# NeSC-IV/sage-icp

Hardware: AMD Instinct MI355X
Metric: ICP frames/sec (120k-pt scan vs 1M-pt map) (higher is better)
Workload: dtype f64

## Files before the change

### sage-icp_amd/csrc/capi_run.hip

```cpp
#include "capi_internal.h"

namespace sageicp_impl {

Rccl g_rccl;
static std::mutex g_rccl_mu;


int load_rccl() {
    std::lock_guard<std::mutex> lk(g_rccl_mu);
    if (g_rccl.h) return SAGEICP_OK;
    const char *names[] = {"librccl.so.1", "librccl.so", "/opt/rocm/lib/librccl.so.1"};
    void *h = nullptr;
    for (const char *n : names) {
        h = dlopen(n, RTLD_NOW | RTLD_NOLOAD | RTLD_GLOBAL);
        if (h) break;
    }
    for (int i = 0; i < 3 && !h; ++i) h = dlopen(names[i], RTLD_NOW | RTLD_GLOBAL);
    if (!h) return fail(SAGEICP_ERR_RCCL, std::string("cannot load librccl: ") + dlerror());
    g_rccl.GetUniqueId = reinterpret_cast<decltype(g_rccl.GetUniqueId)>(dlsym(h, "ncclGetUniqueId"));
    g_rccl.CommInitRank = reinterpret_cast<decltype(g_rccl.CommInitRank)>(dlsym(h, "ncclCommInitRank"));
    g_rccl.CommDestroy = reinterpret_cast<decltype(g_rccl.CommDestroy)>(dlsym(h, "ncclCommDestroy"));
    g_rccl.AllReduce = reinterpret_cast<decltype(g_rccl.AllReduce)>(dlsym(h, "ncclAllReduce"));
    g_rccl.GetErrorString = reinterpret_cast<decltype(g_rccl.GetErrorString)>(dlsym(h, "ncclGetErrorString"));
    g_rccl.CommCount = reinterpret_cast<decltype(g_rccl.CommCount)>(dlsym(h, "ncclCommCount"));
// ... 262 lines not shown
        HIPCHK(hipStreamSynchronize(s));
        return SAGEICP_OK;
    }
    int order_frame() const {
        if (n > 0 && n < static_cast<uint64_t>(std::max(0, env_int("SAGEICP_SORT_FROM", kSortFrameFrom))))
            HIPCHK(check_copy_frame(d_frame, sc.d_sorted.data(), static_cast<int>(n), sc.d_state.data(), comm == nullptr, s));
        else if (n > 0)
            HIPCHK(sort_frame(d_frame, sc.d_sorted.data(), static_cast<int>(n), sc.d_state.data(), true, comm == nullptr,
                              m->host.voxel_size, sc.d_keys.data(), sc.d_vals.data(), sc.d_sort_temp.data(),
                              sc.d_sort_temp.capacity(), s));
        return SAGEICP_OK;
    }
};

struct AttemptPlan {
    LoopPlan loop{};
    bool loop_shape = false, use_loop = false, chain = false;
    int lw = 0, chain_grid = 0;
    unsigned loop_waves = 0;
};
static AttemptPlan plan_attempt(const IcpCall &c, const Attempt &a) {
    Scratch &sc = c.sc;
    const sageicp_comm *comm = c.comm;
    const uint64_t n = c.n;
    AttemptPlan p;
    p.loop_shape = (!comm || (c.p2p && !comm->device_shared && env_int("SAGEICP_CHUNKED", 0) == 0)) &&
                   plan_loop(c.m, n, c.sem_th, &p.loop);
    p.lw = p.loop_shape ? p.loop.lw : icp_lw(n, sparse_voxels(c.m));
    p.use_loop = p.loop_shape && !a.no_loop;
    sc.last_fallback = !p.loop_shape ? SAGEICP_LOOP_FALLBACK_DOES_NOT_FIT : (a.no_loop ? SAGEICP_LOOP_FALLBACK_PEER : SAGEICP_LOOP_FALLBACK_NONE);
    if (p.use_loop && sc.loop_cooldown > 0) {
        --sc.loop_cooldown;
        p.use_loop = false;
        sc.last_fallback = SAGEICP_LOOP_FALLBACK_COOLDOWN;
    }
    p.loop_waves = p.use_loop ? static_cast<unsigned>((n + (64u >> p.loop.lw) - 1) / (64u >> p.loop.lw)) : 0u;
    p.chain_grid = n > 0 ? icp_blocks_for(static_cast<int>(n), p.lw) : 0;
    const bool chain_comm = comm && c.p2p && !comm->device_shared && env_int("SAGEICP_CHAIN_COMM", 0) != 0;
    p.chain = !p.loop_shape && (!comm || chain_comm) && c.polled && n > 0 &&
              p.chain_grid / kChainReplicas <= 255 && !a.no_chain && !c.prof2 && env_int("SAGEICP_CHAIN", 1) != 0;
    return p;
}

static bool solver_is_own_launch(const AttemptPlan &p) {
#ifdef SAGE_LOOP_INGRID
    return p.chain;
#else
    return p.chain || p.use_loop;
#endif
}

static LoopParams solver_params(const IcpCall &c, const AttemptPlan &p, double acc_unscale) {
    LoopParams L{};
    L.sh = c.sc.d_loop.data();
    L.st = c.sc.d_state.data();
    L.timeout_ticks = 100000ull * static_cast<unsigned long long>(std::max(1, env_int("SAGEICP_LOOP_TIMEOUT_MS", 50)));
    const int test_ticks = env_int("SAGEICP_LOOP_TIMEOUT_TICKS", 0);
    if (test_ticks) L.timeout_ticks = static_cast<unsigned long long>(test_ticks);
    if (p.chain) {
        L.wgs = p.chain_grid;
        L.copies = kChainReplicas;
        L.progress = c.sc.d_prog;
        L.count_timeout_ticks = std::max<unsigned long long>(L.timeout_ticks, 20ull * 100000ull) * 10ull;
    } else {
        L.nw = p.loop.nw; L.gpw = p.loop.gpw; L.wgs = p.loop.wgs;
        L.copies = kLoopReplicas;
        L.progress = nullptr;
        L.contiguous = env_int("SAGEICP_LOOP_CONTIGUOUS", 0) ? 1 : 0;
        const uint64_t qw = 64u >> p.loop.lw, groups = (c.n + qw - 1) / qw;
        for (int x = 0; x <= 8; ++x) L.xcd_first[x] = static_cast<uint32_t>(groups * x / 8);
        const uint64_t nwg = static_cast<uint64_t>(p.loop.wgs / 8);
        for (int x = 0; x < 8; ++x)
            if (L.contiguous == 1 && (L.xcd_first[x + 1] - L.xcd_first[x] + nwg - 1) / nwg > static_cast<uint64_t>(p.loop.gpw)) L.contiguous = 0;
        L.count_timeout_ticks = L.timeout_ticks;
        L.prio = std::min(3, std::max(0, env_int("SAGEICP_LOOP_PRIO", 3)));
        L.deal = env_int("SAGEICP_LOOP_DEAL", 1) ? 1 : 0;
    }
    if (c.comm) {
        L.shared_loop = 1;
        if (test_ticks == 0) L.timeout_ticks = std::max(L.timeout_ticks, c.xp.timeout_ticks + 100000000ull);
        if (env_int("SAGEICP_LOOP_COUNT_TIMEOUT_RANK", -1) == c.comm->rank)
            L.count_timeout_ticks = static_cast<unsigned long long>(std::max(1, env_int("SAGEICP_LOOP_COUNT_TIMEOUT_TICKS", 1)));
    }
    L.max_iterations = c.max_it;
    L.epoch = ++c.sc.loop_epoch;
    for (int i = 0; i < 7; ++i) L.T0[i] = c.init[i];
    L.acc_unscale = acc_unscale;
    return L;
}

struct SolverGuard {
    Scratch &sc;
    unsigned long long epoch = 0;
    bool armed = false;
    explicit SolverGuard(Scratch &s) : sc(s) {}
    ~SolverGuard() {
        if (!armed) return;
        const unsigned long long word = epoch | 0x8000000000000000ull;
        (void)hipMemcpyAsync(&sc.d_loop.data()->go[0], &word, sizeof(word), hipMemcpyHostToDevice, sc.stream);
        (void)hipStreamSynchronize(sc.stream);
        (void)hipStreamSynchronize(sc.stream2);
    }
    int start(const LoopParams &L, const P2pParams &xp) {
        launch_loop_solve(L, xp, sc.stream2);
        HIPCHK(hipGetLastError());
        epoch = L.epoch;
        armed = true;
        HIPCHK(hipEventRecord(sc.ev_solve, sc.stream2));
        return SAGEICP_OK;
    }
    void disarm() { armed = false; }
    int send_home_now() {
        sc.go_word = epoch | 0x8000000000000000ull;
        HIPCHK(hipMemcpyAsync(&sc.d_loop.data()->go[0], &sc.go_word, sizeof(sc.go_word), hipMemcpyHostToDevice, sc.stream));
        armed = false;
        return SAGEICP_OK;
    }
};

struct AttemptResult {
    bool looped = false;
    bool chain = false;
    bool chain_gave_up = false;
    int lw = 0;
    bool compact_scan = false;
    double us_nn = 0, us_fin = 0;
    uint32_t nn_launches = 0;
};

static int run_one_launch(const IcpCall &c, const AttemptPlan &p, const IcpParams &ip, const LoopParams &L,
                          SolverGuard &guard, AttemptResult &r) {
    Scratch &sc = c.sc;
    hipStream_t s = c.s;
    int rc;
    if (c.prof && (rc = sc.reserve_events(1))) return rc;
    IcpParams lp = ip;
    lp.filter = p.loop.filter ? ip.filter : 0;
    lp.nwaves = p.loop_waves;
    HIPCHK(hipMemsetAsync(sc.d_loop.data(), 0, offsetof(LoopShared, acc32), s));
    if (c.prof) HIPCHK(hipEventRecord(sc.events[1], s));
    launch_loop(lp, L, p.loop.lw, s);
    if (hipPeekAtLastError() == hipSuccess) guard.disarm();
    if (c.prof) HIPCHK(hipEventRecord(sc.events[2], s));
    if (solver_is_own_launch(p)) HIPCHK(hipStreamWaitEvent(s, sc.ev_solve, 0));
    if ((rc = c.fetch_state(lp.nwaves))) return rc;
    const IcpState &st = *sc.h_state.data();
    r.looped = true;
    if ((st.bad_input && !c.comm) || st.exchange_failed) return SAGEICP_OK;
    if (!st.loop_aborted && st.done) {
        if (c.prof) {
            float a = 0;
            (void)hipEventElapsedTime(&a, sc.events[1], sc.events[2]);
            r.us_nn = 1e3 * a;
            r.nn_launches = static_cast<uint32_t>(std::max(1, st.iter));
        }
        return SAGEICP_OK;
    }
    r.looped = false;
    if (st.peer_aborted) {
        sc.last_fallback = SAGEICP_LOOP_FALLBACK_PEER;
    } else {
        sc.loop_cooldown = std::max(0, env_int("SAGEICP_LOOP_COOLDOWN", 256));
        if (env_int("SAGEICP_LOOP_TIMEOUT_TICKS", 0) == 0 && env_int("SAGEICP_LOOP_COUNT_TIMEOUT_RANK", -1) < 0 && sc.loop_derate < 16) ++sc.loop_derate;
        ++sc.loop_timeouts;
        sc.last_fallback = SAGEICP_LOOP_FALLBACK_TIMEOUT;
        static std::atomic<int> told{0};
        if (told.exchange(1) == 0 && env_int("SAGEICP_QUIET", 0) == 0)
            std::fprintf(stderr, "sageicp: a wait inside the one-launch ICP loop timed out (the GPU is shared with other work, or "
                                 "fewer workgroups are resident than planned): this frame goes through the launch-per-iteration "
                                 "loop, the next %d calls of this map too, later plans take %d workgroups fewer "
                                 "(sageicp_map_loop_status() reports the state)\n", sc.loop_cooldown, 32 * sc.loop_derate);
    }
    if ((rc = c.start_state())) return rc;
    if (c.counting) HIPCHK(hipMemsetAsync(sc.d_cand.data(), 0, sizeof(unsigned long long) * 2 * (ip.nwaves + 1), s));
    return SAGEICP_OK;
}

struct Iterations {
    const IcpCall &c;
    SolverGuard &guard;
    AttemptResult &r;
    IcpParams &ip;
    const int lw;
    const bool chain;
    Scratch &sc = c.sc;
    hipStream_t s = c.s;
    FinParams fp{};
    unsigned stripes = 0;
    bool lpt = false;
    uint32_t *st_work = nullptr, *st_sorted = nullptr, *st_iota = nullptr, *st_order = nullptr;

    bool sampled(int iteration) const { return c.prof2 || (c.prof && (iteration & 7) == 4); }
    bool measures(int iteration) const { return lpt && (iteration == 0 || iteration == 3 || iteration == 15); }

    int begin(const LoopParams &L) {
        ip.acc = sc.d_acc.data();
        if (chain) {
            HIPCHK(hipMemsetAsync(sc.d_loop.data(), 0, sizeof(LoopShared), s));
            ip.chain = sc.d_loop.data();
            ip.chain_timeout = L.timeout_ticks;
            ip.chain_epoch = L.epoch;
            ip.digit_limit = std::min(ip.digit_limit, std::ldexp(1.0, 40));
        }
        fp.st = sc.d_state.data();
        fp.partials = nullptr; fp.nparts = 0; fp.standalone = 0;
        fp.acc = ip.acc;
        fp.acc_unscale = 1.0 / ip.acc_scale;
        fp.mode = c.p2p ? 3 : (c.comm ? 1 : 0);
        if (c.p2p) fp.p2p = c.xp;
        stripes = c.n > 0 ? static_cast<unsigned>(icp_stripes_for(static_cast<int>(c.n), lw)) : 0u;
        lpt = stripes >= 16 && stripes <= sc.sort_cap && stripe_sort_temp_bytes(stripes) <= sc.d_sort_temp.capacity() &&
              env_int("SAGEICP_LPT", c.n >= 40000 ? 1 : 0) != 0;
        st_work = sc.d_keys.data(); st_sorted = sc.d_keys.data() + stripes; st_iota = sc.d_vals.data(); st_order = sc.d_vals.data() + stripes;
        if (lpt) stripe_order_init(st_work, st_iota, stripes, s);
        return SAGEICP_OK;
    }
    int enqueue(int slot, int iteration) {
        const bool ev = sampled(iteration);
        if (ev) HIPCHK(hipEventRecord(sc.events[5 * slot + 1], s));
        ip.stripe_work = measures(iteration) ? st_work : nullptr;
        ip.chain_iter = iteration;
        launch_icp(ip, lw, true, s);
        if (chain && iteration == 0 && hipPeekAtLastError() == hipSuccess) guard.disarm();
        if (measures(iteration)) {
            HIPCHK(stripe_order_sort(st_work, st_sorted, st_iota, st_order, stripes, sc.d_sort_temp.data(), sc.d_sort_temp.capacity(), s));
            ip.stripe_order = st_order;
        }
        if (ev) HIPCHK(hipEventRecord(sc.events[5 * slot + 2], s));
        if (chain) return SAGEICP_OK;
        launch_fin(fp, s);
        if (c.comm && !c.p2p) {
            ncclResult_t e = g_rccl.AllReduce(sc.d_state.data()->sums, sc.d_state.data()->sums, kNumSums,
                                              ncclDouble, ncclSum, c.comm->comm, s);
            if (e != ncclSuccess)
                return fail(SAGEICP_ERR_RCCL, std::string("ncclAllReduce: ") +
                                                  (g_rccl.GetErrorString ? g_rccl.GetErrorString(e) : "?"));
            FinParams f2 = fp;
            f2.mode = 2;
            launch_fin(f2, s);
        }
        if (c.prof2) HIPCHK(hipEventRecord(sc.events[5 * slot + 3], s));
        return SAGEICP_OK;
    }
    void harvest(int slot) {
        float a = 0, b = 0;
        (void)hipEventElapsedTime(&a, sc.events[5 * slot + 1], sc.events[5 * slot + 2]);
        if (c.prof2) (void)hipEventElapsedTime(&b, sc.events[5 * slot + 2], sc.events[5 * slot + 3]);
        r.us_nn += 1e3 * a; r.us_fin += 1e3 * b;
        ++r.nn_launches;
    }

    int run_polled() {
        int rc;
        const int depth = std::min(8, std::max(1, env_int("SAGEICP_DEPTH", 4)));
        volatile unsigned long long *word = &sc.h_prog.data()->word;
        int enq = 0;
        unsigned spins = 0;
        unsigned long long idle_word = ~0ull;
        for (;;) {
            const unsigned long long w = *word;
            const int comp = static_cast<int>(w & 0xFFFFFFFFull);
            if (w >> 32) break;
            if (enq < c.max_it && enq - comp < depth) {
                if ((rc = enqueue(enq, enq))) return rc;
                ++enq;
                spins = 0;
                continue;
            }
            __builtin_ia32_pause();
            if ((++spins & 0xFFFFu) == 0) {
                const hipError_t q = hipStreamQuery(s);
                if (q != hipSuccess && q != hipErrorNotReady)
                    return fail(SAGEICP_ERR_HIP, std::string("ICP loop: ") + hipGetErrorString(q));
                if (q == hipSuccess && (*word >> 32) == 0 && enq >= c.max_it)
                    break;
                if (chain && q == hipSuccess) {
                    if (idle_word == *word) break;
                    idle_word = *word;
                } else {
                    idle_word = ~0ull;
                }
            }
        }
// ... 303 lines not shown
```

### sage-icp_amd/csrc/kernels.h

```cpp
#pragma once

#include <hip/hip_runtime.h>

#include "sageicp_types.h"

namespace sageicp {

constexpr int kRowWords = 32;
constexpr int kRowCq = 27, kRowKey = 28, kRowOcc = 31;
constexpr int kRowLdsStride = 36;

struct LoopShared;
struct IcpParams {
    const Point4 *frame;
    int n;
    const IcpState *st;
    int check_done;
    int apply_pose;
    double voxel_size;
    double inv_voxel_size;
    uint32_t *rows;
    const Slot *table;
    uint32_t mask;
    const Point4 *pts;
    uint32_t pts_bytes;
    int filter;
    int flat;
    const uint4 *cand;
    uint32_t cand_bytes;
    const uint32_t *cand_flags;
    double filt_inv_same;
    double filt_inv_diff;
    double filt_slack;
    double sem_th;
    double dist_init;
    double prune_scale;
    unsigned keep_all;
    int32_t *nn_idx;
    double kernel;
    double accept_r2;
    uint2 *nn_prev;
    uint32_t *work;
    long long *acc;
    double digit_limit;
    double acc_scale;
    uint32_t *stripe_work;
    const uint32_t *stripe_order;
    unsigned long long *counters;
    unsigned nwaves;
#ifdef SAGE_ICP_DELAY_PROBE
    unsigned dbg_delay;
    unsigned dbg_repeat;
#endif
    LoopShared *chain;
    int chain_iter;
    unsigned long long chain_timeout;
    unsigned long long chain_epoch;
};

#ifndef SAGE_ICP_WAVES
#define SAGE_ICP_WAVES 4
#endif
constexpr int kIcpWavesPerBlock = SAGE_ICP_WAVES;
int icp_blocks_for(int n, int lw);
size_t icp_lds_bytes(int lw);
void launch_rows(const IcpParams &p, hipStream_t s);
void launch_derive_cand(const Slot *table, uint32_t nslots, const Point4 *pts, uint4 *cand, uint64_t nslots_pts,
                        uint32_t *flags, hipStream_t s);
void launch_icp(const IcpParams &p, int lw, bool fused, hipStream_t s);

struct GnParams {
    const Point4 *src;
    const Point4 *tgt;
    int n;
    double kernel;
    double *partials;
};
int launch_gn(const GnParams &p, hipStream_t s);

constexpr int kAccReplicas = 32;
constexpr int kAccWords = 64;
constexpr int kAccValues = 17;
struct FinParams {
    IcpState *st;
    const double *partials;
    long long *acc;
    double acc_unscale;
    int nparts;
    int mode;
    int standalone;
    P2pParams p2p;
};
void launch_fin(const FinParams &p, hipStream_t s);

#ifndef SAGE_LOOP_REPLICAS
#define SAGE_LOOP_REPLICAS 8
#endif
constexpr int kLoopReplicas = SAGE_LOOP_REPLICAS;
constexpr int kLoopPoseGranules = 25;
constexpr int kChainReplicas = 32;
struct LoopShared {
    long long acc[2][kLoopReplicas][kAccWords];
    unsigned long long pose[32];
    unsigned long long abort_word[16];
    unsigned long long go[16];
    long long acc32[2][kChainReplicas][kAccWords];
};
struct LoopParams {
    LoopShared *sh;
    IcpState *st;
    int nw;
    int gpw;
    int wgs;
    int contiguous;
    uint32_t xcd_first[9];
    unsigned long long timeout_ticks;
    unsigned long long count_timeout_ticks;
    int max_iterations;
    unsigned long long epoch;
    double T0[7];
    double acc_unscale;
    int shared_loop;
    int prio;
    int deal;
    int copies;
    IcpProgress *progress;
};
struct LoopArgs {
    IcpParams P;
    LoopParams L;
};
#ifndef SAGE_LOOP_OCC
#define SAGE_LOOP_OCC 7
#endif
constexpr int kLoopMaxWavesHost = 8;
constexpr int kLoopStripeHost = 4;
constexpr int kLoopStateWords = 24;
size_t loop_lds_bytes(int lw, int nw, int gpw);
int loop_blocks_per_cu(int lw, bool filter, int nw, size_t lds);
void launch_loop(const IcpParams &p, const LoopParams &l, int lw, hipStream_t s);
void launch_loop_solve(const LoopParams &l, const P2pParams &x, hipStream_t s);

constexpr int kMaxPartials = 1 << 16;
constexpr uint64_t kMaxQueries = (1ull << 26) - 4;

void launch_tf(Point4 *pts, int n, const IcpState *st, hipStream_t s);
void launch_scatter_points(const uint32_t *idx, const Point4 *vals, uint32_t n, Point4 *pts,
                           hipStream_t s);
void launch_scatter_slots(const uint32_t *idx, const Slot *vals, uint32_t n, Slot *table,
                          hipStream_t s);
void launch_scatter_u32(const uint32_t *idx, const uint32_t *vals, uint32_t n, uint32_t *dst, hipStream_t s);
void launch_sum_counters(const unsigned long long *c, int n, IcpState *st, hipStream_t s);

struct VdsParams {
    const Point4 *in;
    int n;
    int do_crop;
    double max_range, min_range, label_max_range;
    int n_groups;
    const int *group_counts;
    const int *group_labels;
    double group_vs[8];
    double scale;
    unsigned long long *keys;
    uint32_t *winner;
    uint32_t mask;
    Point4 *tmp;
    uint32_t *slot_of;
    uint32_t *sort_key;
    uint32_t *sort_val;
    int *overflow;
    unsigned long long *out_keys;
};
size_t vds_sort_temp_bytes(int n);
void launch_vds_permute(const Point4 *in, const uint32_t *perm, uint32_t n, Point4 *out, hipStream_t s);
hipError_t voxel_downsample_device(const VdsParams &P, void *sort_temp, size_t sort_temp_bytes,
                                   uint32_t *d_n_kept, Point4 *out, hipStream_t s);

struct DeskewTangent {
    double v[6];
};
void launch_deskew(const Point4 *in, Point4 *out, const double *ts, int n, const DeskewTangent &d, hipStream_t s);

constexpr int kIngestBadTimestamp = 8;
struct IngestArgs {
    const unsigned char *xyz;
    const unsigned char *label;
    unsigned long long xyz_stride, label_stride;
    int xyz_dtype, label_dtype;
    int n;
    const double *ts;
    double *ts_out;
    int *flags;
};
void launch_ingest(const IngestArgs &a, Point4 *out, hipStream_t s);

constexpr int kOccNonFinite = 16;
constexpr int kOccMaxSide = 4096;
struct OccGrid {
    double lo[3], hi[3];
    double x_res, y_res;
    int h, w;
};
struct OccTransform {
    double R[9];
    double t[3];
};
struct OccDecision {
// ... 27 lines not shown
```

### sage-icp_amd/csrc/kernels.hip

```cpp

#include <hip/hip_runtime.h>

#include <algorithm>
#include <cfloat>
#include <cstdlib>
#include <type_traits>
#include <vector>

#ifndef SAGE_ICP_STRIPE
#define SAGE_ICP_STRIPE 8
#endif
#ifndef SAGE_ICP_OCC
#define SAGE_ICP_OCC 6
#endif
#ifndef SAGE_LOOP_DEPTH_FULL
#define SAGE_LOOP_DEPTH_FULL 2
#endif
#ifndef SAGE_LOOP_DEPTH_COMPACT
#define SAGE_LOOP_DEPTH_COMPACT 2
#endif
#define SAGE_LOOP_DEPTH_OF(filt) ((filt) ? SAGE_LOOP_DEPTH_COMPACT : SAGE_LOOP_DEPTH_FULL)

#include "kernels.h"
#include "se3_math.h"
// ... 283 lines not shown
    if (lane == 0)
        (void)__hip_atomic_fetch_add(wgacc + 3 * kCount, static_cast<unsigned long long>(pairs), __ATOMIC_RELAXED, __HIP_MEMORY_SCOPE_WORKGROUP);
}

template <bool COUNTED = false>
__device__ __forceinline__ void wgacc_flush(unsigned long long *wgacc, long long *dst, long long *overflow) {
    const int lane = static_cast<int>(threadIdx.x & 63u);
    const int l = min(lane, static_cast<int>(kWgAccWords) - 1);
    const long long x = static_cast<long long>(wgacc[l]);
    const bool ok = wgacc[kWgAccWords - 1] == 0ull;
    __builtin_amdgcn_fence(__ATOMIC_ACQ_REL, "wavefront");
    if (lane < static_cast<int>(kWgAccWords)) wgacc[lane] = 0ull;
    if constexpr (COUNTED) {
        (void)overflow;
        if (lane <= 3 * kAccValues)
            (void)__hip_atomic_fetch_add(dst + lane, lane == 3 * kAccValues ? (ok ? 1ll : 257ll) : (ok ? x * 256 + 1 : 1ll),
                                         __ATOMIC_RELAXED, __HIP_MEMORY_SCOPE_AGENT);
    } else if (lane < 3 * kAccValues) {
        {
            if (ok) (void)__hip_atomic_fetch_add(dst + lane, x, __ATOMIC_RELAXED, __HIP_MEMORY_SCOPE_AGENT);
            else (void)__hip_atomic_fetch_or(overflow, 1ll, __ATOMIC_RELAXED, __HIP_MEMORY_SCOPE_AGENT);
        }
    }
}

struct LoopGroup {
    uint32_t *rows;
    uint32_t *state;
    const uint32_t *perm;
    uint32_t *work;
    unsigned unit;
    double *red;
    unsigned long long *wgacc;
    unsigned q_first;
    unsigned slot;
#ifdef SAGE_LOOP_TIMING
    unsigned long long ph[8], tprev;
#endif
};
constexpr int kLoopMaxWaves = kLoopMaxWavesHost;
constexpr unsigned kLoopStripe = kLoopStripeHost;
constexpr int kNoVoxel = 0x7FFFFFFF;
constexpr unsigned kStPrev = 16, kStKey = 18;
constexpr unsigned kLpArrive = 0, kLpNext = 1, kLpDone = 2;
constexpr unsigned kLpPose = 4;
constexpr unsigned kLpDbg = kLpPose + 24u;
constexpr unsigned kLpFirst = kLpDbg + 4u;
constexpr unsigned kLpAcc = kLpFirst + 8u;
constexpr unsigned kLpHeaderWords = (kLpAcc + 2u * kWgAccWords + 15u) & ~15u;
__host__ __device__ constexpr unsigned loop_group_words(int lw) {
    return static_cast<unsigned>((kRowLdsStride + kLoopStateWords) * (64 >> lw));
}
__host__ __device__ constexpr unsigned loop_red_words() { return 2u * kCount * 4u; }
__host__ __device__ constexpr unsigned loop_perm_words(unsigned nblk) { return 2u * ((nblk + 7u) & ~7u); }

#ifndef SAGE_LOOP_FLAT_MINW
#define SAGE_LOOP_FLAT_MINW 8
#endif
template <int LW, bool FUSED, bool FILT, bool PERSIST = false, bool FLATQ = false>
__device__ __forceinline__ void icp_body(const IcpParams &P, uint32_t *smem, LoopGroup *G = nullptr,
                                         const double *pose = nullptr);

struct PairCompact {
    uint4 a, b;
    unsigned ka, oa;
    bool ha, hb;
};
struct PairFull {
    Point4 a, b;
    unsigned ka;
    bool ha, hb;
};
struct PairCompactFlat {
    uint4 a, b;
    unsigned ka, oa, kb, ob;
    bool ha, hb;
};
struct PairFullFlat {
    Point4 a, b;
    unsigned ka, kb;
    bool ha, hb;
};

__device__ __forceinline__ void chain_wait_pose(const IcpParams &P, uint32_t *smem, int lane) {
    LoopShared *sh = P.chain;
    const unsigned long long tag = static_cast<unsigned long long>(P.chain_iter);
    const unsigned long long *src = lane < kLoopPoseGranules ? &sh->pose[lane] : &sh->abort_word[0];
    const unsigned long long t0 = __builtin_amdgcn_s_memrealtime();
    unsigned go = 0u;
    unsigned long long g;
    for (;;) {
        g = ld_agent(src);
        const unsigned long long g24 = static_cast<unsigned long long>(static_cast<unsigned>(__builtin_amdgcn_readlane(static_cast<int>(g), 24))) |
                                       (static_cast<unsigned long long>(static_cast<unsigned>(__builtin_amdgcn_readlane(static_cast<int>(g >> 32), 24))) << 32);
        const bool ok = lane >= kLoopPoseGranules || (g >> 32) == tag;
        if (__all(ok)) {
            if (static_cast<uint32_t>(g24) != 0u) go = 1u;
            break;
        }
        if ((g24 >> 32) < tag && static_cast<uint32_t>(g24) != 0u) {
            go = 1u;
            break;
        }
        const bool late = __builtin_amdgcn_s_memrealtime() - t0 > P.chain_timeout;
        if (__any(lane == kLoopPoseGranules && g != 0ull) || late) {
            if (lane == 0 && late) {
                st_agent(&sh->abort_word[0], 1ull);
                const_cast<IcpState *>(P.st)->loop_aborted = 1;
            }
            go = 2u;
            break;
        }
        __builtin_amdgcn_s_sleep(8);
    }
    if (!go && lane < 24) smem[kWgPose + static_cast<unsigned>(lane)] = static_cast<uint32_t>(g);
    if (lane == 0) smem[kWgGo] = go;
}

template <int LW, bool FUSED, bool FILT, bool FLATQ>
__global__ __launch_bounds__(64 * kIcpWavesPerBlock) __attribute__((amdgpu_waves_per_eu(SAGE_ICP_OCC, 8)))
void k_icp(IcpParams P) {
    extern __shared__ __attribute__((aligned(16))) uint32_t smem[];
    if (P.chain) {
        if (P.chain_iter == 0) {
            const bool bad = P.st->done != 0;
            if (blockIdx.x == 0 && threadIdx.x == 0) st_agent(&P.chain->go[0], P.chain_epoch | (bad ? 0x8000000000000000ull : 0ull));
            if (bad) return;
        }
    } else if (P.check_done && P.st->done) {
        return;
    }
    icp_body<LW, FUSED, FILT, false, FLATQ>(P, smem);
    PROBE_DELAY_REPEAT((icp_body<LW, FUSED, FILT, false, FLATQ>(P, smem)));
}

template <int LW, bool FUSED, bool FILT, bool PERSIST, bool FLATQ>
__device__ __forceinline__ void icp_body(const IcpParams &P, uint32_t *smem, LoopGroup *G, const double *pose) {
    static_assert(!PERSIST || FUSED, "the persistent loop always accumulates");
    constexpr int W = 1 << LW;
    constexpr int QW = 64 >> LW;
    constexpr int SH = 5;
    PROBE_NN_BEGIN;
    PROBE_DELAY_BEGIN;
    int lane;
    if constexpr (PERSIST) {
        unsigned l;
        asm volatile("v_mbcnt_lo_u32_b32 %0, -1, 0\n\tv_mbcnt_hi_u32_b32 %0, -1, %0" : "=v"(l));
        lane = static_cast<int>(l);
    } else {
        lane = static_cast<int>(threadIdx.x & 63u);
    }
    const int wv = __builtin_amdgcn_readfirstlane(static_cast<int>(threadIdx.x >> 6));
    if (FUSED && !PERSIST) {
        if (threadIdx.x == 0) {
            smem[kWgArrive] = 0u;
            smem[kWgGo] = 0u;
        }
        if (threadIdx.x < 2u * kWgAccWords) smem[kWgAcc + threadIdx.x] = 0u;
        if (threadIdx.x < 12u && !(P.chain && P.chain_iter > 0))
            reinterpret_cast<double *>(smem + kWgPose)[threadIdx.x] = threadIdx.x < 9u ? P.st->R[threadIdx.x] : P.st->T[4u + threadIdx.x - 9u];
        __syncthreads();
    }
    uint32_t *wl;
    if constexpr (PERSIST) wl = G->rows;
    else wl = smem + kWgHeaderWords + static_cast<unsigned>(wv) * icp_wave_words(LW);

    constexpr unsigned kStripe = SAGE_ICP_STRIPE;
    unsigned wave_id, stripe_id = 0u;
    if constexpr (PERSIST) {
        wave_id = G->slot;
// ... 932 lines not shown
#define LOOP_STAMP_WG(it, k) do { if ((it) < kLoopTimedIters && blockIdx.x < kLoopTimedWgs && (threadIdx.x & 63u) == 0u) g_loop_wg[it][blockIdx.x][k] = __builtin_amdgcn_s_memrealtime(); } while (0)
extern "C" void sageicp_debug_loop_phases(unsigned long long *out, int reset) {
    (void)hipMemcpyFromSymbol(out, HIP_SYMBOL(g_loop_phase), sizeof(unsigned long long) * 16);
    if (reset) {
        unsigned long long z[16] = {0};
        (void)hipMemcpyToSymbol(HIP_SYMBOL(g_loop_phase), z, sizeof(z));
    }
}
extern "C" void sageicp_debug_loop_waves(unsigned long long *out) {
    (void)hipMemcpyFromSymbol(out, HIP_SYMBOL(g_loop_wave), sizeof(unsigned long long) * kLoopTimedIters * kLoopTimedWgs * 8 * 2);
}
extern "C" void sageicp_debug_loop_info(unsigned *info) {
    (void)hipMemcpyFromSymbol(info, HIP_SYMBOL(g_loop_wginfo), sizeof(unsigned) * kLoopTimedIters * kLoopTimedWgs * 4);
}
extern "C" void sageicp_debug_loop_times(unsigned long long *wg, unsigned long long *solver) {
    (void)hipMemcpyFromSymbol(wg, HIP_SYMBOL(g_loop_wg), sizeof(unsigned long long) * kLoopTimedIters * kLoopTimedWgs * 4);
    (void)hipMemcpyFromSymbol(solver, HIP_SYMBOL(g_loop_solver), sizeof(unsigned long long) * kLoopTimedIters * 4);
}
#else
#define LOOP_STAMP_SOLVER(it, k) do { } while (0)
#define LOOP_STAMP_SOLVER2(it, k) do { } while (0)
#define LOOP_STAMP_WG(it, k) do { } while (0)
#endif


__device__ __forceinline__ int exchange_sums_wave(double *S, const P2pParams &X, unsigned long long g) {
    const int lane = static_cast<int>(threadIdx.x & 63u);
    const int slot = static_cast<int>(g & 1ull);
    const unsigned long long tag = g + 1ull;
    if (lane < kNumSums) {
        const double v = S[lane];
        for (int r = 0; r < X.nranks; ++r)
            __hip_atomic_store(&X.block[r]->sums[slot][X.rank][lane], v, __ATOMIC_RELAXED, __HIP_MEMORY_SCOPE_SYSTEM);
    }
    asm volatile("s_waitcnt vmcnt(0)" ::: "memory");
    __builtin_amdgcn_fence(__ATOMIC_RELEASE, "");
    asm volatile("s_waitcnt vmcnt(0)" ::: "memory");
    if (lane == 0)
        for (int r = 0; r < X.nranks; ++r)
            __hip_atomic_store(&X.block[r]->flag[X.rank], tag, __ATOMIC_RELAXED, __HIP_MEMORY_SCOPE_SYSTEM);
    P2pBlock *mine = X.block[X.rank];
    bool late = false, gone = false;
    if (lane < X.nranks) {
        const unsigned long long t0 = __builtin_amdgcn_s_memrealtime();
        while (__hip_atomic_load(&mine->flag[lane], __ATOMIC_RELAXED, __HIP_MEMORY_SCOPE_SYSTEM) < tag) {
            __builtin_amdgcn_s_sleep(2);
            if (__builtin_amdgcn_s_memrealtime() - t0 > X.timeout_ticks) {
                late = true;
                break;
            }
        }
        __builtin_amdgcn_fence(__ATOMIC_ACQUIRE, "");
        gone = __hip_atomic_load(&mine->abort_tag[lane], __ATOMIC_RELAXED, __HIP_MEMORY_SCOPE_SYSTEM) == tag;
    }
    late = __any(late);
    gone = __any(gone);
    __builtin_amdgcn_fence(__ATOMIC_ACQUIRE, "");
    if (lane < kNumSums) {
        double s = 0.0;
        for (int r = 0; r < X.nranks; ++r)
            s += __hip_atomic_load(&mine->sums[slot][r][lane], __ATOMIC_RELAXED, __HIP_MEMORY_SCOPE_SYSTEM);
        S[lane] = s;
    }
    __builtin_amdgcn_wave_barrier();
    return gone ? 2 : (late ? 1 : 0);
}
__device__ __forceinline__ void exchange_abort_wave(const P2pParams &X, unsigned long long g) {
    const int lane = static_cast<int>(threadIdx.x & 63u);
    if (lane == 0)
        for (int r = 0; r < X.nranks; ++r)
            __hip_atomic_store(&X.block[r]->abort_tag[X.rank], g + 1ull, __ATOMIC_RELAXED, __HIP_MEMORY_SCOPE_SYSTEM);
    asm volatile("s_waitcnt vmcnt(0)" ::: "memory");
    __builtin_amdgcn_fence(__ATOMIC_RELEASE, "");
    asm volatile("s_waitcnt vmcnt(0)" ::: "memory");
    if (lane == 0)
        for (int r = 0; r < X.nranks; ++r)
            __hip_atomic_store(&X.block[r]->flag[X.rank], g + 1ull, __ATOMIC_RELAXED, __HIP_MEMORY_SCOPE_SYSTEM);
    asm volatile("s_waitcnt vmcnt(0)" ::: "memory");
}

struct SolveLds {
    double T[14];
    double S[kNumSums];
    double pub[12];
    long long digits[kAccWords];
};
template <int COPIES>
__device__ __forceinline__ unsigned loop_finish_iteration(const LoopParams &L, const P2pParams &X, SolveLds &m, int it,
                                                          unsigned long long &xg) {
    LoopShared *sh = L.sh;
    IcpState *st = L.st;
    const int lane = static_cast<int>(threadIdx.x & 63u);
    double *sT = m.T, *S = m.S, *pub = m.pub;
    long long *digits = m.digits;
    const unsigned long long tag = static_cast<unsigned long long>(it) + 1ull;

    {
        const long long per = static_cast<long long>(L.wgs / COPIES);
        long long (*acc)[kAccWords] = COPIES == kLoopReplicas ? sh->acc[it & 1] : sh->acc32[it & 1];
        long long v[COPIES];
        const unsigned long long t0 = __builtin_amdgcn_s_memrealtime();
        for (;;) {
#pragma unroll
            for (int r = 0; r < COPIES; ++r)
                v[r] = __hip_atomic_load(&acc[r][lane], __ATOMIC_RELAXED, __HIP_MEMORY_SCOPE_AGENT);
            bool ok = true;
            if (lane <= 3 * kAccValues) {
#pragma unroll
                for (int r = 0; r < COPIES; ++r) ok &= (v[r] & 255ll) == per;
            }
            if (__all(ok)) break;
            unsigned long long ab = 0ull;
            if (lane == 0) ab = ld_agent(&sh->abort_word[0]);
            const bool late = __builtin_amdgcn_s_memrealtime() - t0 > L.count_timeout_ticks;
            if (__any(ab != 0ull) || late) {
                if (lane == 0) {
                    st_agent(&sh->abort_word[0], 1ull);
                    st->loop_aborted = 1;
                    st_agent(&sh->pose[24], (tag << 32) | 2ull);
                    if (L.progress)
                        __hip_atomic_store(&L.progress->word, (1ull << 32) | static_cast<unsigned long long>(it), __ATOMIC_RELAXED,
                                           __HIP_MEMORY_SCOPE_SYSTEM);
                }
                if (X.nranks > 1) {
                    exchange_abort_wave(X, xg);
                    xg += 1ull;
                    if (lane == 0) *X.exchanges = xg;
                }
                return 2u;
            }
            __builtin_amdgcn_s_sleep(1);
        }
        LOOP_STAMP_SOLVER(it, 0);
        long long d = 0;
        if (lane <= 3 * kAccValues) {
#pragma unroll
            for (int r = 0; r < COPIES; ++r) d += (v[r] - per) >> 8;
        }
#pragma unroll
        for (int r = 0; r < COPIES; ++r)
            __hip_atomic_store(&acc[r][lane], 0ll, __ATOMIC_RELAXED, __HIP_MEMORY_SCOPE_AGENT);
        digits[lane] = d;
        __builtin_amdgcn_wave_barrier();
        if (lane < kNumSums) {
            double r = 0.0;
            if (lane < kAccValues) {
                const double a = static_cast<double>(digits[3 * lane]);
                const double b = static_cast<double>(digits[3 * lane + 1]);
                const double c = static_cast<double>(digits[3 * lane + 2]);
                r = a + (b * 9.094947017729282e-13 + c * 8.271806125530277e-25);
                if (lane < kCount) r *= L.acc_unscale;
            }
            S[lane] = r;
        }
        __builtin_amdgcn_wave_barrier();
    }
    const bool overflow = digits[3 * kAccValues] != 0;
    LOOP_STAMP_SOLVER(it, 1);

    bool exchange_failed = false;
    if (X.nranks > 1) {
        const int ex = exchange_sums_wave(S, X, xg);
        xg += 1ull;
        if (lane == 0) *X.exchanges = xg;
        exchange_failed = ex == 1;
        if (ex == 2) {
            if (lane == 0) {
                st_agent(&sh->abort_word[0], 1ull);
                st->loop_aborted = 1;
                st->peer_aborted = 1;
                st_agent(&sh->pose[24], (tag << 32) | 2ull);
                if (L.progress)
                    __hip_atomic_store(&L.progress->word, (1ull << 32) | static_cast<unsigned long long>(it), __ATOMIC_RELAXED,
                                       __HIP_MEMORY_SCOPE_SYSTEM);
            }
            return 2u;
        }
    }

    double x[6], est[7], nrm;
    solve_normal_equations_t<WaveLanes>(S, x);
    LOOP_STAMP_SOLVER2(it, 0);
    se3_exp_sqrt_t<WaveLanes>(x, est, SAGE_SQNORM6(x), nrm);
    LOOP_STAMP_SOLVER2(it, 1);
    double rhs[7], Tn[7];
    {
        const double *src = sT + (lane == 1 ? 7 : 0);
#pragma unroll
        for (int i = 0; i < 7; ++i) rhs[i] = src[i];
    }
    se3_mul(est, rhs, Tn);
    __builtin_amdgcn_wave_barrier();
    if (lane < 2) {
        double *dst = sT + (lane == 1 ? 7 : 0);
#pragma unroll
        for (int i = 0; i < 7; ++i) dst[i] = Tn[i];
    }
    double Rn[9];
    quat_to_mat(Tn, Rn);
    LOOP_STAMP_SOLVER2(it, 2);
    if (!(x[3] * x[3] + x[4] * x[4] + x[5] * x[5] < 9.0) || fabs(nrm - kEstimationThreshold) < 1e-12) {
        double lg[6];
        se3_log(est, lg);
        nrm = sqrt(SAGE_SQNORM6(lg));
    }
    LOOP_STAMP_SOLVER2(it, 3);
    const bool converged = nrm < kEstimationThreshold;
    unsigned done = (converged || it + 1 >= L.max_iterations) ? 1u : 0u;
    if (overflow && !L.shared_loop) done = 1u;
    if (exchange_failed) done = 1u;
    if (lane == 0) {
#pragma unroll
        for (int i = 0; i < 9; ++i) pub[i] = Rn[i];
        pub[9] = Tn[4]; pub[10] = Tn[5]; pub[11] = Tn[6];
    }
    __builtin_amdgcn_wave_barrier();
    LOOP_STAMP_SOLVER(it, 2);
    asm volatile("s_waitcnt vmcnt(0)" ::: "memory");
    if (lane < 24) st_agent(&sh->pose[lane], (tag << 32) | reinterpret_cast<const uint32_t *>(pub)[lane]);
    if (lane == 24) st_agent(&sh->pose[24], (tag << 32) | done);
    if (lane == 0) {
        if (it < kHistory) st->n_corr[it] = static_cast<uint32_t>(S[kCount]);
        if (overflow) st->acc_overflow = 1;
        if (exchange_failed) st->exchange_failed = 1;
        if (done) {
#pragma unroll
            for (int i = 0; i < 7; ++i) st->T[i] = Tn[i];
#pragma unroll
            for (int i = 0; i < 9; ++i) st->R[i] = Rn[i];
            st->last_step_norm = nrm;
            st->iter = it + 1;
            st->done = 1;
            st->converged = (converged && !exchange_failed) ? 1 : 0;
        }
    }
    if (done && lane == 1) {
#pragma unroll
        for (int i = 0; i < 7; ++i) st->T_icp[i] = Tn[i];
    }
    if (L.progress && lane == 0)
        __hip_atomic_store(&L.progress->word, (static_cast<unsigned long long>(done ? 1u : 0u) << 32) | static_cast<unsigned long long>(it + 1),
                           __ATOMIC_RELAXED, __HIP_MEMORY_SCOPE_SYSTEM);
    if (done && lane < kNumSums) st->sums[lane] = S[lane];
    LOOP_STAMP_SOLVER(it, 3);
    return done;
}

struct SolveArgs {
    LoopParams L;
    P2pParams X;
};
template <int COPIES>
__global__ __launch_bounds__(64) void k_loop_solve(SolveArgs A) {
    __shared__ SolveLds m;
    __builtin_amdgcn_s_setprio(3);
    {
        const int lane = static_cast<int>(threadIdx.x & 63u);
        const unsigned long long t0 = __builtin_amdgcn_s_memrealtime();
        for (;;) {
            const unsigned long long g = ld_agent(&A.L.sh->go[0]);
            if ((g & 0x7FFFFFFFFFFFFFFFull) == A.L.epoch) {
                if (g >> 63) return;
                break;
            }
            if (__builtin_amdgcn_s_memrealtime() - t0 > 1000ull * A.L.timeout_ticks + 1000000000ull) {
                if (lane == 0) A.L.st->loop_aborted = 1;
                return;
            }
            __builtin_amdgcn_s_sleep(32);
        }
        if (lane < 14) m.T[lane] = lane < 7 ? A.L.T0[lane] : (lane == 10 ? 1.0 : 0.0);
    }
    unsigned long long xg = A.X.nranks > 1 ? *A.X.exchanges : 0ull;
    __builtin_amdgcn_wave_barrier();
    for (int it = 0;; ++it) {
        auto ka = __builtin_amdgcn_kernarg_segment_ptr();
        asm volatile("" : "+s"(ka));
        const SolveArgs &K = *(const SolveArgs *)(ka);
        if (loop_finish_iteration<COPIES>(K.L, K.X, m, it, xg)) return;
    }
}

#ifndef SAGE_LOOP_POLL_SLEEP
#define SAGE_LOOP_POLL_SLEEP 8
#endif
template <int LW, bool FILT>
__global__ __launch_bounds__(64 * kLoopMaxWaves) __attribute__((amdgpu_waves_per_eu(SAGE_LOOP_OCC, 8)))
void k_loop(LoopArgs A) {
    extern __shared__ __attribute__((aligned(16))) uint32_t smem[];
    constexpr int QW = 64 >> LW;
    const IcpParams &P = A.P;
    const LoopParams &L = A.L;
    const int wv = __builtin_amdgcn_readfirstlane(static_cast<int>(threadIdx.x >> 6));
    const int nw = L.nw;
    const unsigned gpw = static_cast<unsigned>(L.gpw);
    double *s_pose = reinterpret_cast<double *>(smem + kLpPose);

    {
        const bool bad = !L.shared_loop && P.st->bad_input;
        if (blockIdx.x == 0 && threadIdx.x == 0)
            st_agent(&L.sh->go[0], L.epoch | (bad ? 0x8000000000000000ull : 0ull));
        if (bad) return;
    }
// ... 139 lines not shown
            G.rows = rows;
            G.state = state;
            G.perm = perm;
            G.work = work;
            G.unit = gi;
            G.red = red;
            G.wgacc = wgacc;
            G.q_first = g0 * QW;
            G.slot = g0 + gi;
#ifdef SAGE_LOOP_TIMING
            for (int i = 0; i < 8; ++i) G.ph[i] = 0;
            G.tprev = __builtin_amdgcn_s_memtime();
            ++n_pass;
#endif
            {
                auto kb = __builtin_amdgcn_kernarg_segment_ptr();
                asm volatile("" : "+s"(kb));
                icp_body<LW, true, FILT, true>(((const LoopArgs *)(kb))->P, smem, &G, s_pose);
            }
#ifdef SAGE_LOOP_TIMING
            if (gi >= static_cast<unsigned>(nw)) LOOP_STAMP_WG(it, 3);
            if (it < kLoopTimedIters && blockIdx.x < kLoopTimedWgs && lane == 0 && wv < 8 && gi < static_cast<unsigned>(nw)) {
                unsigned hw;
                asm volatile("s_getreg_b32 %0, hwreg(HW_REG_HW_ID)" : "=s"(hw));
                g_loop_wave[it][blockIdx.x][wv][0] = __builtin_amdgcn_s_memrealtime();
                g_loop_wave[it][blockIdx.x][wv][1] = (t_unit << 24) | (static_cast<unsigned long long>(gi & 0xFFu) << 16) | (hw & 0xFFFFu);
            }
#endif
#ifdef SAGE_LOOP_TIMING
            for (int i = 0; i < 8; ++i) ph[i] += G.ph[i];
#endif
        }
#ifdef SAGE_LOOP_TIMING
        const unsigned long long t_a = __builtin_amdgcn_s_memtime();
#endif
        unsigned prior = 0u;
        __atomic_signal_fence(__ATOMIC_SEQ_CST);
        if (lane == 0)
            prior = __hip_atomic_fetch_add(&smem[kLpArrive], 1u, __ATOMIC_RELAXED, __HIP_MEMORY_SCOPE_WORKGROUP);
        __atomic_signal_fence(__ATOMIC_SEQ_CST);
        prior = static_cast<unsigned>(__builtin_amdgcn_readfirstlane(static_cast<int>(prior)));
        const bool last = prior == static_cast<unsigned>(nw) - 1u;
        if (last) {
            wgacc_flush<true>(wgacc, &sh->acc[it & 1][blockIdx.x & (kLoopReplicas - 1)][0], &sh->acc[it & 1][0][kAccWords - 1]);
            if (lane == 0) {
                smem[kLpArrive] = 0u;
                smem[kLpNext] = L.deal ? static_cast<unsigned>(nw) : 0u;
            }
            if (nblk <= 64u && nblk > BPW) {
                __builtin_amdgcn_fence(__ATOMIC_ACQ_REL, "wavefront");
                const unsigned i = static_cast<unsigned>(lane);
                const unsigned wi = i < nblk ? work[i] : 0u;
                unsigned rank = 0u;
                for (unsigned j = 0; j < nblk; ++j) {
                    const unsigned wj = work[j];
                    rank += (wj > wi || (wj == wi && j < i)) ? 1u : 0u;
                }
                __builtin_amdgcn_fence(__ATOMIC_ACQ_REL, "wavefront");
                if (i < nblk) {
                    perm[rank] = i;
                    work[i] = 0u;
                }
            }
#ifdef SAGE_LOOP_TIMING
            if (lane == 0 && it < kLoopTimedIters && blockIdx.x < kLoopTimedWgs) {
                unsigned hw;
                asm volatile("s_getreg_b32 %0, hwreg(HW_REG_HW_ID)" : "=s"(hw));
                unsigned xcc;
                asm volatile("s_getreg_b32 %0, hwreg(HW_REG_XCC_ID)" : "=s"(xcc));
                unsigned *o = g_loop_wginfo[it][blockIdx.x];
                o[0] = (xcc << 28) | (hw & 0x0FFFFFFFu);
                o[1] = smem[kLpDbg]; o[2] = smem[kLpDbg + 1]; o[3] = smem[kLpDbg + 2];
                smem[kLpDbg] = 0u; smem[kLpDbg + 1] = 0u; smem[kLpDbg + 2] = 0u;
            }
#endif
            LOOP_STAMP_WG(it, 0);
        }
        if (wv == 0) {
            const unsigned long long tag = static_cast<unsigned long long>(it) + 1ull;
            const unsigned long long t0 = __builtin_amdgcn_s_memrealtime();
            unsigned long long g = tag << 32;
            bool aborted = false;
            for (;;) {
                if (lane < kLoopPoseGranules) g = ld_agent(&sh->pose[lane]);
                const bool ok = (g >> 32) == tag;
                if (__all(ok)) break;
                unsigned long long ab = 0ull;
                if (lane == 0) ab = ld_agent(&sh->abort_word[0]);
                const bool late = __builtin_amdgcn_s_memrealtime() - t0 > L.timeout_ticks;
                if (__any(ab != 0ull) || late) {
                    if (lane == 0 && late) {
                        st_agent(&sh->abort_word[0], 1ull);
                        L.st->loop_aborted = 1;
                    }
                    aborted = true;
                    break;
                }
                __builtin_amdgcn_s_sleep(SAGE_LOOP_POLL_SLEEP);
                if (L.wgs > 1024) __builtin_amdgcn_s_sleep(SAGE_LOOP_POLL_SLEEP);
            }
            if (aborted) {
                if (lane == 0) smem[kLpDone] = 2u;
            } else {
                if (lane < 24) reinterpret_cast<uint32_t *>(s_pose)[lane] = static_cast<uint32_t>(g);
                if (lane == 24) smem[kLpDone] = static_cast<uint32_t>(g);
            }
            LOOP_STAMP_WG(it, 1);
        }
#ifdef SAGE_LOOP_TIMING
        const unsigned long long t_b = __builtin_amdgcn_s_memtime();
        if (last) t_close += t_b - t_a;
#endif
        __syncthreads();
#ifdef SAGE_LOOP_TIMING
        t_wait += __builtin_amdgcn_s_memtime() - t_b;
#endif
        if (smem[kLpDone]) break;
    }
#ifdef SAGE_LOOP_TIMING
    if ((threadIdx.x & 63u) == 0u) {
        for (int i = 0; i < 8; ++i) atomicAdd(&g_loop_phase[i], ph[i]);
        atomicAdd(&g_loop_phase[8], t_wait);
        atomicAdd(&g_loop_phase[9], t_close);
        atomicAdd(&g_loop_phase[10], n_pass);
    }
#endif
}

__global__ __launch_bounds__(256) void k_gn(GnParams P) {
    __shared__ double red[kCount][16 * 17];
    double acc[kCount];
#pragma unroll
    for (int i = 0; i < kCount; ++i) acc[i] = 0.0;
    const double k = P.kernel;
    const double k2 = k * k;
    const int stride = gridDim.x * 256;
    for (int q = blockIdx.x * 256 + threadIdx.x; q < P.n; q += stride) {
        const Point4 s = P.src[q], g = P.tgt[q];
        const double sx = s.x, sy = s.y, sz = s.z;
        const double rx = sx - g.x, ry = sy - g.y, rz = sz - g.z;
        const double r2 = SAGE_SQNORM3_RESID(rx * rx, ry * ry, rz * rz);
        const double den = k + r2;
        const double w = k2 / (den * den);
        const double wsx = w * sx, wsy = w * sy, wsz = w * sz;
        acc[kW] += w;
        acc[kWsx] += wsx; acc[kWsy] += wsy; acc[kWsz] += wsz;
        acc[kWxx] += wsx * sx; acc[kWxy] += wsx * sy; acc[kWxz] += wsx * sz;
        acc[kWyy] += wsy * sy; acc[kWyz] += wsy * sz; acc[kWzz] += wsz * sz;
        acc[kWrx] += w * rx; acc[kWry] += w * ry; acc[kWrz] += w * rz;
        acc[kWcx] += w * (sy * rz - sz * ry);
        acc[kWcy] += w * (sz * rx - sx * rz);
        acc[kWcz] += w * (sx * ry - sy * rx);
    }
    const int t = static_cast<int>(threadIdx.x);
    const int slot = (t >> 4) * 17 + (t & 15);
#pragma unroll
    for (int c = 0; c < kCount; ++c) red[c][slot] = acc[c];
    __syncthreads();
    const double *row = &red[t >> 4][(t & 15) * 17];
    double v = row[0];
#pragma unroll
    for (int i = 1; i < 16; ++i) v += row[i];
    v += dpp_f64<kDppXor1>(v);
    v += dpp_f64<kDppXor2>(v);
    v += dpp_f64<kDppHalfMirror>(v);
    v += dpp_f64<kDppMirror>(v);
    double *out = P.partials + static_cast<size_t>(blockIdx.x) * kNumSums;
// ... 237 lines not shown
```

Baseline: 212.9.

## Replicate published pose across eight copies and move digit reduction into registers

The solver wave now writes the per-iteration pose words into eight separate cache-line copies, and each workgroup polls the copy picked by its block index. This spreads the spin-wait traffic of all workgroups across several lines instead of one hot line. It also replaces the LDS staging of the accumulator digits and the published pose with cross-lane shuffles and readlane, which removes LDS round trips and wave barriers from the solver's critical path. The cost is more stores per iteration and an extra addressing mode controlled by an environment variable.

```diff
diff --git a/profiles/chain_hops.py b/profiles/chain_hops.py
--- /dev/null
+++ b/profiles/chain_hops.py
@@ -0,0 +1,62 @@
+import ctypes as C
+import os
+import sys
+
+sys.path.insert(0, os.getcwd())
+import numpy as np
+import sage_icp_amd as sage
+
+sage.LIB_PATH = os.environ.get("LOOP_LIB", os.path.join(os.path.dirname(sage.LIB_PATH), "_probe", "libsageicp_looptiming.so"))
+from sage_icp_amd import synthetic as syn
+
+name = sys.argv[1] if len(sys.argv) > 1 else "c2"
+p = syn.PARAMS["cold"]
+w = syn.make_workload(name, lambda: sage.VoxelHashMap(syn.WORKLOADS[name]["voxel"], 100.0))
+f = sage.Frame(w["map"], w["scan"])
+os.environ["SAGEICP_LOOP"] = "2"
+sage.set_counting(False)
+for _ in range(3):
+    pose, st = sage.register_frame(f, w["map"], sage.IDENTITY, p["max_dist"], p["kernel"], p["sem_th"], return_stats=True)
+assert st.single_launch == 1
+IT, WG = 32, 2048
+wg = np.zeros((IT, WG, 4), dtype=np.uint64)
+sv = np.zeros((IT, 4), dtype=np.uint64)
+s2 = np.zeros((IT, 4), dtype=np.uint64)
+sage.lib().sageicp_debug_loop_times(wg.ctypes.data_as(C.c_void_p), sv.ctypes.data_as(C.c_void_p))
+sage.lib().sageicp_debug_loop_solver2(s2.ctypes.data_as(C.c_void_p))
+wg = wg.astype(np.float64) / 100.0
+sv = sv.astype(np.float64) / 100.0
+s2 = s2.astype(np.float64) / 100.0
+used = wg[1, :, 0] > 0
+n = min(IT, st.iterations) - 1
+its = list(range(3, n))
+print("%s: %d queries, %d lanes/query, %d iterations, %d workgroups; iterations 3..%d of an instrumented build, us"
+      % (name, len(w["scan"]), st.lanes_per_query, st.iterations, int(used.sum()), n - 1))
+period = np.diff(sv[3:n, 2])
+print("iteration period (ready to publish -> the next): mean %.2f  p0 %.2f  p50 %.2f  p100 %.2f  | change from one to the next: p50 %.2f p90 %.2f p100 %.2f"
+      % (period.mean(), period.min(), np.median(period), period.max(),
+         np.median(np.abs(np.diff(period))), np.quantile(np.abs(np.diff(period)), .9), np.abs(np.diff(period)).max()))
+
+
+def line(label, a):
+    a = np.asarray(a)
+    print("   %-52s mean %.2f  p0 %.2f  p50 %.2f  p90 %.2f  p100 %.2f" % (label, a.mean(), a.min(), np.median(a), np.quantile(a, .9), a.max()))
+
+
+last_in = np.array([wg[i, used, 0].max() for i in its])
+line("last workgroup counted in -> solver saw the counts", sv[its, 0] - last_in)
+line("counts complete -> sums in fp64", sv[its, 1] - sv[its, 0])
+line("solve", s2[its, 0] - sv[its, 1])
+line("exponential", s2[its, 1] - s2[its, 0])
+line("composition + rotation matrix", s2[its, 2] - s2[its, 1])
+line("composition -> ready to publish (norm test, hand-over)", sv[its, 2] - s2[its, 2])
+line("ready to publish -> stores issued, history written", sv[its, 3] - sv[its, 2])
+line("counts complete -> ready to publish", sv[its, 2] - sv[its, 0])
+held = np.stack([wg[i, used, 1] - sv[i, 2] for i in its])
+print("   ready to publish -> pose held by a workgroup (per iteration's percentile, mean over iterations):")
+print("      all      p0 %.2f  p50 %.2f  p90 %.2f  p100 %.2f" % (held.min(1).mean(), np.median(held, 1).mean(), np.quantile(held, .9, 1).mean(), held.max(1).mean()))
+b = np.arange(WG)[used]
+for x in range(8):
+    h = held[:, (b & 7) == x]
+    print("      XCD %d    p0 %.2f  p50 %.2f  p90 %.2f  p100 %.2f" % (x, h.min(1).mean(), np.median(h, 1).mean(), np.quantile(h, .9, 1).mean(), h.max(1).mean()))
+line("last workgroup counted in -> last workgroup holds the pose", np.array([wg[i, used, 1].max() for i in its]) - last_in)
diff --git a/sage-icp_amd/csrc/capi_run.hip b/sage-icp_amd/csrc/capi_run.hip
--- a/sage-icp_amd/csrc/capi_run.hip
+++ b/sage-icp_amd/csrc/capi_run.hip
@@ -368,6 +368,7 @@
         if (env_int("SAGEICP_LOOP_COUNT_TIMEOUT_RANK", -1) == c.comm->rank)
             L.count_timeout_ticks = static_cast<unsigned long long>(std::max(1, env_int("SAGEICP_LOOP_COUNT_TIMEOUT_TICKS", 1)));
     }
+    L.pose_map = std::min(2, std::max(0, env_int("SAGEICP_LOOP_POSE_MAP", 0)));
     L.max_iterations = c.max_it;
     L.epoch = ++c.sc.loop_epoch;
     for (int i = 0; i < 7; ++i) L.T0[i] = c.init[i];
@@ -485,6 +486,7 @@
             HIPCHK(hipMemsetAsync(sc.d_loop.data(), 0, sizeof(LoopShared), s));
             ip.chain = sc.d_loop.data();
             ip.chain_timeout = L.timeout_ticks;
+            ip.chain_pose_map = L.pose_map;
             ip.chain_epoch = L.epoch;
             ip.digit_limit = std::min(ip.digit_limit, std::ldexp(1.0, 40));
         }
diff --git a/sage-icp_amd/csrc/kernels.h b/sage-icp_amd/csrc/kernels.h
--- a/sage-icp_amd/csrc/kernels.h
+++ b/sage-icp_amd/csrc/kernels.h
@@ -54,6 +54,7 @@
 #endif
     LoopShared *chain;
     int chain_iter;
+    int chain_pose_map;
     unsigned long long chain_timeout;
     unsigned long long chain_epoch;
 };
@@ -98,10 +99,12 @@
 #endif
 constexpr int kLoopReplicas = SAGE_LOOP_REPLICAS;
 constexpr int kLoopPoseGranules = 25;
+constexpr int kLoopPoseCopies = 8;
+constexpr int kLoopPoseStride = 32;
 constexpr int kChainReplicas = 32;
 struct LoopShared {
     long long acc[2][kLoopReplicas][kAccWords];
-    unsigned long long pose[32];
+    unsigned long long pose[kLoopPoseCopies][kLoopPoseStride];
     unsigned long long abort_word[16];
     unsigned long long go[16];
     long long acc32[2][kChainReplicas][kAccWords];
@@ -124,6 +127,7 @@
     int prio;
     int deal;
     int copies;
+    int pose_map;
     IcpProgress *progress;
 };
 struct LoopArgs {
diff --git a/sage-icp_amd/csrc/kernels.hip b/sage-icp_amd/csrc/kernels.hip
--- a/sage-icp_amd/csrc/kernels.hip
+++ b/sage-icp_amd/csrc/kernels.hip
@@ -389,10 +389,14 @@
     bool ha, hb;
 };
 
+__device__ __forceinline__ unsigned loop_pose_copy(int pose_map) {
+    const unsigned b = blockIdx.x;
+    return pose_map == 1 ? 0u : ((pose_map == 2 ? b + 3u : b) & static_cast<unsigned>(kLoopPoseCopies - 1));
+}
 __device__ __forceinline__ void chain_wait_pose(const IcpParams &P, uint32_t *smem, int lane) {
     LoopShared *sh = P.chain;
     const unsigned long long tag = static_cast<unsigned long long>(P.chain_iter);
-    const unsigned long long *src = lane < kLoopPoseGranules ? &sh->pose[lane] : &sh->abort_word[0];
+    const unsigned long long *src = lane < kLoopPoseGranules ? &sh->pose[loop_pose_copy(P.chain_pose_map)][lane] : &sh->abort_word[0];
     const unsigned long long t0 = __builtin_amdgcn_s_memrealtime();
     unsigned go = 0u;
     unsigned long long g;
@@ -1491,19 +1495,28 @@
 struct SolveLds {
     double T[14];
     double S[kNumSums];
-    double pub[12];
-    long long digits[kAccWords];
 };
+__device__ __forceinline__ unsigned long long readlane_u64(unsigned long long v, int src) {
+    const unsigned lo = static_cast<unsigned>(__builtin_amdgcn_readlane(static_cast<int>(static_cast<unsigned>(v)), src));
+    const unsigned hi = static_cast<unsigned>(__builtin_amdgcn_readlane(static_cast<int>(static_cast<unsigned>(v >> 32)), src));
+    return (static_cast<unsigned long long>(hi) << 32) | lo;
+}
+__device__ __forceinline__ int lane_now() {
+    unsigned l;
+    asm volatile("v_mbcnt_lo_u32_b32 %0, -1, 0\n\tv_mbcnt_hi_u32_b32 %0, -1, %0" : "=v"(l));
+    return static_cast<int>(l);
+}
 template <int COPIES>
 __device__ __forceinline__ unsigned loop_finish_iteration(const LoopParams &L, const P2pParams &X, SolveLds &m, int it,
                                                           unsigned long long &xg) {
     LoopShared *sh = L.sh;
     IcpState *st = L.st;
     const int lane = static_cast<int>(threadIdx.x & 63u);
-    double *sT = m.T, *S = m.S, *pub = m.pub;
-    long long *digits = m.digits;
+    double *sT = m.T, *S = m.S;
     const unsigned long long tag = static_cast<unsigned long long>(it) + 1ull;
 
+    double sum = 0.0;
+    bool overflow;
     {
         const long long per = static_cast<long long>(L.wgs / COPIES);
         long long (*acc)[kAccWords] = COPIES == kLoopReplicas ? sh->acc[it & 1] : sh->acc32[it & 1];
@@ -1526,11 +1539,11 @@
                 if (lane == 0) {
                     st_agent(&sh->abort_word[0], 1ull);
                     st->loop_aborted = 1;
-                    st_agent(&sh->pose[24], (tag << 32) | 2ull);
                     if (L.progress)
                         __hip_atomic_store(&L.progress->word, (1ull << 32) | static_cast<unsigned long long>(it), __ATOMIC_RELAXED,
                                            __HIP_MEMORY_SCOPE_SYSTEM);
                 }
+                if (const int al = lane_now(); al < kLoopPoseCopies) st_agent(&sh->pose[al][24], (tag << 32) | 2ull);
                 if (X.nranks > 1) {
                     exchange_abort_wave(X, xg);
                     xg += 1ull;
@@ -1549,22 +1562,19 @@
 #pragma unroll
         for (int r = 0; r < COPIES; ++r)
             __hip_atomic_store(&acc[r][lane], 0ll, __ATOMIC_RELAXED, __HIP_MEMORY_SCOPE_AGENT);
-        digits[lane] = d;
+        const int sl = lane_now();
+        const int s3 = 3 * (sl < kAccValues ? sl : 0);
+        const double a = static_cast<double>(__shfl(d, s3));
+        const double b = static_cast<double>(__shfl(d, s3 + 1));
+        const double c = static_cast<double>(__shfl(d, s3 + 2));
+        if (lane < kAccValues) {
+            sum = a + (b * 9.094947017729282e-13 + c * 8.271806125530277e-25);
+            if (lane < kCount) sum *= L.acc_unscale;
+        }
+        if (lane < kNumSums) S[lane] = sum;
+        overflow = readlane_u64(static_cast<unsigned long long>(d), 3 * kAccValues) != 0ull;
         __builtin_amdgcn_wave_barrier();
-        if (lane < kNumSums) {
-            double r = 0.0;
-            if (lane < kAccValues) {
-                const double a = static_cast<double>(digits[3 * lane]);
-                const double b = static_cast<double>(digits[3 * lane + 1]);
-                const double c = static_cast<double>(digits[3 * lane + 2]);
-                r = a + (b * 9.094947017729282e-13 + c * 8.271806125530277e-25);
-                if (lane < kCount) r *= L.acc_unscale;
-            }
-            S[lane] = r;
-        }
-        __builtin_amdgcn_wave_barrier();
-    }
-    const bool overflow = digits[3 * kAccValues] != 0;
+    }
     LOOP_STAMP_SOLVER(it, 1);
 
     bool exchange_failed = false;
@@ -1578,11 +1588,11 @@
                 st_agent(&sh->abort_word[0], 1ull);
                 st->loop_aborted = 1;
                 st->peer_aborted = 1;
-                st_agent(&sh->pose[24], (tag << 32) | 2ull);
                 if (L.progress)
                     __hip_atomic_store(&L.progress->word, (1ull << 32) | static_cast<unsigned long long>(it), __ATOMIC_RELAXED,
                                        __HIP_MEMORY_SCOPE_SYSTEM);
             }
+            if (const int al = lane_now(); al < kLoopPoseCopies) st_agent(&sh->pose[al][24], (tag << 32) | 2ull);
             return 2u;
         }
     }
@@ -1618,16 +1628,21 @@
     unsigned done = (converged || it + 1 >= L.max_iterations) ? 1u : 0u;
     if (overflow && !L.shared_loop) done = 1u;
     if (exchange_failed) done = 1u;
-    if (lane == 0) {
-#pragma unroll
-        for (int i = 0; i < 9; ++i) pub[i] = Rn[i];
-        pub[9] = Tn[4]; pub[10] = Tn[5]; pub[11] = Tn[6];
-    }
-    __builtin_amdgcn_wave_barrier();
+    const int pl = lane_now();
+    const int gl = (pl & 31) - 2;
+    uint32_t word = done;
+#pragma unroll
+    for (int i = 0; i < 12; ++i) {
+        const unsigned long long v = static_cast<unsigned long long>(__double_as_longlong(i < 9 ? Rn[i] : Tn[i - 5]));
+        if ((gl >> 1) == i) word = static_cast<uint32_t>((gl & 1) ? v >> 32 : v);
+    }
     LOOP_STAMP_SOLVER(it, 2);
     asm volatile("s_waitcnt vmcnt(0)" ::: "memory");
-    if (lane < 24) st_agent(&sh->pose[lane], (tag << 32) | reinterpret_cast<const uint32_t *>(pub)[lane]);
-    if (lane == 24) st_agent(&sh->pose[24], (tag << 32) | done);
+    if (gl >= 0 && gl < kLoopPoseGranules) {
+#pragma unroll
+        for (int c = 0; c < kLoopPoseCopies; c += 2)
+            st_agent(&sh->pose[c + (pl >> 5)][gl], (tag << 32) | word);
+    }
     if (lane == 0) {
         if (it < kHistory) st->n_corr[it] = static_cast<uint32_t>(S[kCount]);
         if (overflow) st->acc_overflow = 1;
@@ -1933,7 +1948,7 @@
             unsigned long long g = tag << 32;
             bool aborted = false;
             for (;;) {
-                if (lane < kLoopPoseGranules) g = ld_agent(&sh->pose[lane]);
+                if (lane < kLoopPoseGranules) g = ld_agent(&sh->pose[loop_pose_copy(L.pose_map)][lane]);
                 const bool ok = (g >> 32) == tag;
                 if (__all(ok)) break;
                 unsigned long long ab = 0ull;
```

Measured after the change: 218.9 (median of 6 runs). 2.8% higher.
